# RIVM-bioinformatics/TrueConsense

Hardware: NVIDIA B200
Metric: aligned_bases_per_sec_pileup_consensus (higher is better)
Workload: dtype int32

## Files before the change

trueconsense_b200/csrc/cuda/pileup_warp.cu:

```cuda
#include <limits.h>

#include "pileup_smem.cuh"

namespace {

using namespace tcsm;
constexpr int HI_PLANES = 7;
constexpr int RUN_CAP = 2047;
#ifndef TC_CHUNK_WORDS
#define TC_CHUNK_WORDS 6
#endif
constexpr int CHUNK_WORDS = TC_CHUNK_WORDS;
#ifndef TC_MAX_WARPS
#define TC_MAX_WARPS 24
#endif
#ifndef TC_CIG_PER_WC
#define TC_CIG_PER_WC 15
#endif
#ifndef TC_SEQ_PER_WC
#define TC_SEQ_PER_WC 26
#endif
#ifndef TC_TMA_STAGING
#define TC_TMA_STAGING 1
#endif
#ifndef TC_STAGE_UNROLL
#define TC_STAGE_UNROLL 4
#endif
#ifndef TC_PHASE_WORDS
#define TC_PHASE_WORDS 32
#endif
template <int WC> struct geom {
    static constexpr int ROWW = WC * 8;
    static constexpr int PW = (TC_PHASE_WORDS > 0 && TC_PHASE_WORDS < WC) ? TC_PHASE_WORDS : WC;
    static constexpr int NPH = WC / PW;
    static constexpr int NW = WC / 32;
    static constexpr int RS = PW + 1;
    static constexpr int SEQ_PAD = 4;
    static constexpr int SEQ_CAP = WC * TC_SEQ_PER_WC;
    static constexpr int CIG_CAP = WC * TC_CIG_PER_WC;
    static constexpr int SEQ_WORDS = SEQ_PAD + SEQ_CAP + 8;
    static constexpr int CIG_WORDS = CIG_CAP / 2 + 4;
    static constexpr int WARP_WORDS = 32 * RS + SEQ_WORDS + CIG_WORDS;
    static constexpr int WARPS = (227 * 1024 / 4) / (WARP_WORDS + 2) > TC_MAX_WARPS ? TC_MAX_WARPS : (227 * 1024 / 4) / (WARP_WORDS + 2);
    static constexpr bool TMA = TC_TMA_STAGING && (CIG_CAP + 4 <= 32 * RS);
};

extern __shared__ __align__(16) uint32_t smem[];

struct lane_walk {
    uint32_t cp, cend;
    uint32_t c0, c1;
    uint32_t prev;
    int x, y, rem;
};

template <int ROWW, int CW, bool LIMIT>
__device__ __forceinline__ bool emit_phase(lane_walk& s, const int lq, const uint32_t rowp, const int xlim,
                                           unsigned long long* xi, const int xi_n, const uint32_t sq, int* err) {
    bool any_iter = false;
    while (__any_sync(FULL, (s.cp < s.cend || s.rem > 0) && (!LIMIT || s.x < xlim))) {
        any_iter = true;
        if (s.rem == 0 && s.cp < s.cend && (!LIMIT || s.x < xlim)) {
            uint32_t c = s.c0;
            uint32_t fl = op_flags(c & 15u);
            if (!(fl & 1u)) {
                const uint32_t op = c & 15u;
                const int l = (int)(c >> 4);
                const bool is_d = (op == OP_D);
                const bool ev = is_d || (op == OP_I && (s.prev & 2u));
                const uint32_t col = (uint32_t)min(is_d ? s.x : s.x - 1, xi_n - 1);
                const uint32_t pd = s.prev & 1u;
                red_xi_if(ev, xi, col, is_d ? 1u : 0u - pd, (is_d ? 1u : pd) ^ 1u);
                if (is_d && l > 1) for (int k = s.x + 1; k < min(s.x + l, xi_n); ++k) red_xi_if(true, xi, (uint32_t)k, 1u, 0u);
                s.prev = (fl & 2u) | (is_d ? 1u : 0u);
                if (fl & 2u) s.x += l;
                if (fl & 4u) s.y += l;
                s.cp += 2;
                c = s.c1;
                fl = op_flags(c & 15u);
            }
            if ((fl & 1u) && s.cp < s.cend) {
                const int l = (int)(c >> 4);
                if (s.x + l > ROWW || s.y + l > lq) { atomicCAS(err, 0, TC_ERR_CAPACITY); s.cp = s.cend; }
                else { s.rem = l; s.cp += 2; }
            }
            s.c0 = lds16(s.cp); s.c1 = lds16(s.cp + 2);
        }
        __syncwarp();
        if (s.rem > 0 && (!LIMIT || s.x < xlim)) {
            const int x = s.x;
            const int kb = x & 7;
            const int cl = LIMIT ? min(min(s.rem, 8 * CW - kb), xlim - x) : min(s.rem, 8 * CW - kb);
            {
                const int q0 = (x - kb) + (s.y - x);
                const uint32_t src = sq + (uint32_t)((q0 >> 3) << 2);
                const int sh4 = (q0 & 7) << 2;
                uint32_t w[CW + 1];
#pragma unroll
                for (int j = 0; j <= CW; ++j) w[j] = lds(src + 4 * j);
                const int rem4 = 4 * (kb + cl);
                const uint32_t ro = rowp + (uint32_t)((x >> 3) << 2);
                reds_or(ro, __funnelshift_l(w[1], w[0], sh4) & (0xffffffffu >> (4 * kb)) & ~__funnelshift_rc(0xffffffffu, 0u, rem4));
#pragma unroll
                for (int j = 1; j < CW; ++j)
                    reds_or(ro + 4 * j, __funnelshift_l(w[j + 1], w[j], sh4) & ~__funnelshift_rc(0xffffffffu, 0u, max(rem4 - 32 * j, 0)));
            }
            s.x += cl; s.y += cl; s.rem -= cl;
            s.prev = 2u;
        }
    }
    return any_iter;
}

template <int WC, bool PIECES>
__global__ void __launch_bounds__(geom<WC>::WARPS * 32, 1) warp_pileup_kernel(pileup_args a) {
    using G = geom<WC>;
    constexpr int ROWW = G::ROWW, RS = G::RS, NW = G::NW, NPH = G::NPH, PW = G::PW, KW = G::PW / 32;
    const int lane = threadIdx.x & 31;
    const int L = a.L;
    if (PIECES && a.status->err) return;

    const bool fold = !PIECES && a.span_hint > 0;
    const int ms = PIECES ? PIECE_COLS : ((max(fold ? a.span_hint : a.status->max_span, 1) + 7) & ~7);
    const int slack32 = (256 - ms - 8) & ~7, slack64 = (512 - ms - 8) & ~7, slack128 = (1024 - ms - 8) & ~7;
    const bool mine = (WC == 32) ? (slack32 >= MIN_SLACK)
                    : (WC == 64) ? (slack32 < MIN_SLACK && slack64 >= MIN_SLACK) : (slack64 < MIN_SLACK);
    if (!mine) return;
    const int slack = (WC == 32) ? slack32 : (WC == 64) ? slack64 : slack128;
    if (slack < MIN_SLACK) {
        if (threadIdx.x == 0 && blockIdx.x == 0) atomicCAS(&a.status->err, 0, TC_ERR_CAPACITY);
        return;
    }

    const uint32_t rows = (uint32_t)__cvta_generic_to_shared(smem) + 4u * (threadIdx.x >> 5) * G::WARP_WORDS;
    const uint32_t seq_s = rows + 4u * 32 * RS;
    const uint32_t cig_s = seq_s + 4u * G::SEQ_WORDS;
    for (int i = lane; i < 32 * RS; i += 32) sts(rows + 4 * i, 0u);
    if (lane < G::SEQ_PAD) sts(seq_s + 4 * lane, 0u);
    const uint32_t mbar = (uint32_t)__cvta_generic_to_shared(smem) + 4u * G::WARPS * G::WARP_WORDS + 8u * (threadIdx.x >> 5);
    uint32_t tma_parity = 0;
    if (G::TMA && lane == 0) { mbar_init(mbar, 1); asm volatile("fence.mbarrier_init.release.cluster;" ::: "memory"); }
    __syncwarp();

    const int64_t n_reads = PIECES ? a.n_pieces : a.r.n;
    const int64_t n_seq_words = (int64_t)a.r.seq_off[a.r.n];
    const int64_t n_ops_total = PIECES ? 0 : (int64_t)a.r.cigar_off[a.r.n];
    const int64_t gw = (int64_t)blockIdx.x * G::WARPS + (threadIdx.x >> 5);
    const int64_t n_warps = (int64_t)gridDim.x * G::WARPS;
    int64_t r = gw * n_reads / n_warps;
    const int64_t r_end = (gw + 1) * n_reads / n_warps;

    uint32_t ones[NW], twos[NW], fours[NW], eights[NW], hi[NW][HI_PLANES];
#pragma unroll
    for (int j = 0; j < NW; ++j) {
        ones[j] = twos[j] = fours[j] = eights[j] = 0;
#pragma unroll
        for (int p = 0; p < HI_PLANES; ++p) hi[j][p] = 0;
    }
    int w0 = INT_MIN, run_reads = 0;
    const uint32_t row = rows + 4u * lane * RS;
    int prev_pos = (fold && r > 0 && r < r_end) ? a.r.pos[r - 1] : INT_MIN;
    int my_max_span = 0, my_zero_span = 0;

    auto flush = [&]() {
        __syncwarp();
#pragma unroll
        for (int j = 0; j < NW; ++j) {
            uint32_t planes[4 + HI_PLANES];
            planes[0] = ones[j]; planes[1] = twos[j]; planes[2] = fours[j]; planes[3] = eights[j];
#pragma unroll
            for (int p = 0; p < HI_PLANES; ++p) planes[4 + p] = hi[j][p];
            uint32_t any = 0;
#pragma unroll
            for (int p = 0; p < 4 + HI_PLANES; ++p) any |= planes[p];
            if (any) {
#pragma unroll 4
                for (int bit = 0; bit < 32; ++bit) {
                    if (!((any >> bit) & 1u)) continue;
                    int v = 0;
#pragma unroll
                    for (int p = 0; p < 4 + HI_PLANES; ++p) v |= (int)((planes[p] >> bit) & 1u) << p;
                    const int colr = w0 + 8 * (lane + 32 * j) + (7 - (bit >> 2));
                    const int cls = bit & 3;
                    const int crow = cls == 0 ? TC_ROW_A : cls == 1 ? TC_ROW_C : cls == 2 ? TC_ROW_G : TC_ROW_T;
                    if (colr < L) atomicAdd(&a.counts[(size_t)crow * L + colr], v);
                }
            }
            ones[j] = twos[j] = fours[j] = eights[j] = 0;
#pragma unroll
            for (int p = 0; p < HI_PLANES; ++p) hi[j][p] = 0;
        }
        __syncwarp();
    };

    while (r < r_end) {
        const int nmax = (int)min((int64_t)32, r_end - r);
        const bool valid = lane < nmax;
        const int64_t ri = r + (valid ? lane : 0);
        int p, lq, n, nops_lane, y0 = 0;
        bool passes = true, declined = false;
        uint32_t big = 0;
        uint32_t cs, sq_lane;
        if constexpr (PIECES) {
            const tc_piece* pc = a.pieces + a.piece_order[ri];
            const uint4 m0 = __ldg(reinterpret_cast<const uint4*>(pc)), m1 = __ldg(reinterpret_cast<const uint4*>(pc) + 1);
            p = (int)m0.x; lq = (int)m1.y; y0 = (int)m1.z;
            passes = p < L;
            const uint32_t so = m0.y, co = m0.z;
            nops_lane = (int)m0.w;
            const int p0 = __shfl_sync(FULL, p, 0);
            const bool fresh = (w0 == INT_MIN);
            if (fresh) w0 = max(p0, 0) & ~7;
            const int sv = (int)(((so & 3u) + m1.x + 3u) >> 2), cv = (int)(((co & 3u) + m0.w + 3u) >> 2);
            int s_inc = valid ? sv : 0, c_inc = valid ? cv : 0;
#pragma unroll
            for (int o = 1; o < 32; o <<= 1) {
                const int ts = __shfl_up_sync(FULL, s_inc, o), tc = __shfl_up_sync(FULL, c_inc, o);
                if (lane >= o) { s_inc += ts; c_inc += tc; }
            }
            const bool inwin = p >= w0 && p - w0 < slack;
            const bool fits = valid && inwin && 4 * s_inc <= G::SEQ_CAP && 4 * c_inc <= G::CIG_CAP;
            const unsigned fm = __ballot_sync(FULL, fits);
            n = (fm == FULL) ? 32 : __ffs(~fm) - 1;
            n = min(n, RUN_CAP - run_reads);
            if (n == 0) {
                const bool inwin0 = __shfl_sync(FULL, (int)inwin, 0) != 0;
                if ((!inwin0 && !fresh) || run_reads >= RUN_CAP) {
                    flush();
                    w0 = INT_MIN; run_reads = 0;
                    continue;
                }
                if (lane == 0) atomicCAS(&a.status->err, 0, TC_ERR_CAPACITY);
                r += 1;
                continue;
            }
            const uint32_t sdst = seq_s + 4u * G::SEQ_PAD + 16u * (uint32_t)(s_inc - sv);
            const uint32_t cdst = cig_s + 8u * (uint32_t)(c_inc - cv);
            const int64_t sb_p = (int64_t)(so & ~3u);
            const bool tma_p = G::TMA && __all_sync(FULL, lane >= n || sb_p + 4ll * sv <= n_seq_words);
            if (tma_p) {
                const int s_tot = __shfl_sync(FULL, s_inc, n - 1), c_tot = __shfl_sync(FULL, c_inc, n - 1);
                fence_proxy_async();
                __syncwarp();
                if (lane == 0) mbar_expect_tx(mbar, 16u * (uint32_t)(s_tot + c_tot));
                __syncwarp();
                if (lane < n) {
                    tma_bulk_g2s(sdst, a.r.seq4 + sb_p, 16u * (uint32_t)sv, mbar);
                    if (cv > 0) tma_bulk_g2s(rows + 16u * (uint32_t)(c_inc - cv), a.r.cigar + (co & ~3u), 16u * (uint32_t)cv, mbar);
                }
                mbar_wait(mbar, tma_parity);
                tma_parity ^= 1u;
                const uint32_t sbase = seq_s + 4u * G::SEQ_PAD;
                for (int i = lane; i < s_tot; i += 32) {
                    uint4 v = lds4(sbase + 16 * i);
                    if (multibit(v.x) | multibit(v.y) | multibit(v.z) | multibit(v.w)) {
                        v.x = clear_multibit(v.x); v.y = clear_multibit(v.y); v.z = clear_multibit(v.z); v.w = clear_multibit(v.w);
                    }
                    v.x = __byte_perm(v.x, 0, 0x0123); v.y = __byte_perm(v.y, 0, 0x0123);
                    v.z = __byte_perm(v.z, 0, 0x0123); v.w = __byte_perm(v.w, 0, 0x0123);
                    sts4(sbase + 16 * i, v);
                }
                for (int i = lane; i < c_tot; i += 32) {
                    const uint4 v0 = lds4(rows + 16 * i);
                    big |= v0.x | v0.y | v0.z | v0.w;
                    sts2(cig_s + 8 * i, pack_ops(v0.x, v0.y), pack_ops(v0.z, v0.w));
                    sts4(rows + 16 * i, make_uint4(0u, 0u, 0u, 0u));
                }
            } else {
                if (lane < n) {
                    const int64_t sb = (int64_t)(so & ~3u);
                    constexpr int SB = 4;
                    const bool whole = sb + 4ll * sv <= n_seq_words;
                    for (int v0 = 0; v0 < sv; v0 += SB) {
                        uint4 q[SB];
    #pragma unroll
                        for (int u = 0; u < SB; ++u) {
                            const int v = v0 + u;
                            if (v < sv) {
                                if (whole) q[u] = __ldg(reinterpret_cast<const uint4*>(a.r.seq4 + sb) + v);
                                else {
                                    q[u].x = sb + 4 * v + 0 < n_seq_words ? __ldg(a.r.seq4 + sb + 4 * v + 0) : 0u;
                                    q[u].y = sb + 4 * v + 1 < n_seq_words ? __ldg(a.r.seq4 + sb + 4 * v + 1) : 0u;
                                    q[u].z = sb + 4 * v + 2 < n_seq_words ? __ldg(a.r.seq4 + sb + 4 * v + 2) : 0u;
                                    q[u].w = sb + 4 * v + 3 < n_seq_words ? __ldg(a.r.seq4 + sb + 4 * v + 3) : 0u;
                                }
                            }
                        }
    #pragma unroll
                        for (int u = 0; u < SB; ++u) {
                            const int v = v0 + u;
                            if (v < sv) {
                                if (multibit(q[u].x) | multibit(q[u].y) | multibit(q[u].z) | multibit(q[u].w)) {
                                    q[u].x = clear_multibit(q[u].x); q[u].y = clear_multibit(q[u].y); q[u].z = clear_multibit(q[u].z); q[u].w = clear_multibit(q[u].w);
                                }
                                q[u].x = __byte_perm(q[u].x, 0, 0x0123); q[u].y = __byte_perm(q[u].y, 0, 0x0123);
                                q[u].z = __byte_perm(q[u].z, 0, 0x0123); q[u].w = __byte_perm(q[u].w, 0, 0x0123);
                                sts4(sdst + 16 * v, q[u]);
                            }
                        }
                    }
                    const uint4* csrc = reinterpret_cast<const uint4*>(a.r.cigar + (co & ~3u));
                    for (int v0 = 0; v0 < cv; v0 += 4) {
                        uint4 q[4];
    #pragma unroll
                        for (int u = 0; u < 4; ++u) if (v0 + u < cv) q[u] = __ldg(csrc + v0 + u);
    #pragma unroll
                        for (int u = 0; u < 4; ++u)
                            if (v0 + u < cv) {
                                big |= q[u].x | q[u].y | q[u].z | q[u].w;
                                sts2(cdst + 8 * (v0 + u), pack_ops(q[u].x, q[u].y), pack_ops(q[u].z, q[u].w));
                            }
                    }
                }
            }
            __syncwarp();
            cs = cdst + 2u * (co & 3u);
            if (__any_sync(FULL, big >= OP_BIG)) {
                if (lane < n) {
                    bool after_sat = false;
                    for (uint32_t k = 0; k < m0.w; ++k) {
                        const uint32_t c = __ldg(a.r.cigar + co + k), op = c & 15u;
                        if (c >= OP_BIG) {
                            if (op == OP_H) sts16(cs + 2 * k, (1u << 4) | OP_H);
                            else if (op == OP_S) { sts16(cs + 2 * k, S_SATURATED); after_sat = true; }
                            else declined = true;
                        } else if (after_sat && op_flags(op) != 0u) declined = true;
                    }
                }
                __syncwarp();
            }
            sq_lane = sdst + 4u * (so & 3u);
        } else {
            p = a.r.pos[ri];
            const uint32_t so = a.r.seq_off[ri], so_next = a.r.seq_off[ri + 1];
            const uint32_t co = a.r.cigar_off[ri], co_next = a.r.cigar_off[ri + 1];
            const uint32_t flg = a.r.flag[ri];
            lq = a.r.l_seq[ri];
            passes = !(flg & (a.flag_filter | 4u)) && !(a.ignore_orphans && (flg & 1u) && !(flg & 2u));
            if (a.min_mapq > 0 && a.r.mapq && (int)a.r.mapq[ri] < a.min_mapq) passes = false;
            if (p >= L) {
                if (fold && valid && passes) atomicCAS(&a.status->err, 0, TC_ERR_RANGE);
                passes = false;
            }
            const int p0 = __shfl_sync(FULL, p, 0);
            const bool fresh = (w0 == INT_MIN);
            if (fresh) w0 = max(p0, 0) & ~7;
            const uint32_t sbase_al = __shfl_sync(FULL, so, 0) & ~3u;
            const uint32_t cbase_al = __shfl_sync(FULL, co, 0) & ~3u;
            const bool inwin = p >= w0 && p - w0 < slack;
            const bool fits = valid && inwin && (so_next - sbase_al + 1 <= (uint32_t)G::SEQ_CAP) && (co_next - cbase_al <= (uint32_t)G::CIG_CAP);
            const unsigned fm = __ballot_sync(FULL, fits);
            n = (fm == FULL) ? 32 : __ffs(~fm) - 1;
            n = min(n, RUN_CAP - run_reads);
            if (n == 0) {
                const bool inwin0 = __shfl_sync(FULL, (int)inwin, 0) != 0;
                if ((!inwin0 && !fresh) || run_reads >= RUN_CAP) {
                    flush();
                    w0 = INT_MIN; run_reads = 0;
                    continue;
                }
                if (inwin0 && lane == 0) atomicCAS(&a.status->err, 0, TC_ERR_CAPACITY);
                if (fold && lane == 0) {
                    if (p0 < prev_pos) atomicCAS(&a.status->err, 0, TC_ERR_UNSORTED);
                    if (p0 < 0 && passes) atomicCAS(&a.status->err, 0, TC_ERR_RANGE);
                }
                prev_pos = p0;
                r += 1;
                continue;
            }

            {
                const uint32_t send = __shfl_sync(FULL, so_next, n - 1) + 1;
                const int nv = (int)((send - sbase_al + 3) >> 2);
                const uint32_t cend = __shfl_sync(FULL, co_next, n - 1);
                const int ncv = (int)((cend - cbase_al + 3) >> 2);
                uint32_t dirty = 0;
                const uint32_t sdst = seq_s + 4u * G::SEQ_PAD;
                uint32_t exmin = 1u;
                const bool use_tma = G::TMA && (int64_t)sbase_al + 4ll * nv <= n_seq_words && (int64_t)cbase_al + 4ll * ncv <= n_ops_total;
                if (use_tma) {
                    fence_proxy_async();
                    __syncwarp();
                    if (lane == 0) {
                        mbar_expect_tx(mbar, 16u * (uint32_t)(nv + ncv));
                        tma_bulk_g2s(sdst, a.r.seq4 + sbase_al, 16u * (uint32_t)nv, mbar);
                        if (ncv > 0) tma_bulk_g2s(rows, a.r.cigar + cbase_al, 16u * (uint32_t)ncv, mbar);
                    }
                }
                {
                    const int64_t s_lo = ((int64_t)send - 1) & ~3ll, s_len = (int64_t)send - sbase_al;
                    const int64_t c_lo = (int64_t)cend & ~3ll, c_len = (int64_t)cend - cbase_al;
                    if (lane == 0) {
                        const int64_t sw = min(s_len + 4, n_seq_words - s_lo) & ~3ll, cw = min(c_len + 4, n_ops_total - c_lo) & ~3ll;
                        if (sw > 0) prefetch_l2_bulk(a.r.seq4 + s_lo, (uint32_t)(4 * sw));
                        if (cw > 0) prefetch_l2_bulk(a.r.cigar + c_lo, (uint32_t)(4 * cw));
                    }
                    const int64_t rm = r + n + 64;
                    if (rm < n_reads) {
                        if (lane == 0) prefetch_l2(a.r.pos + rm);
                        if (lane == 1) prefetch_l2(a.r.seq_off + rm);
                        if (lane == 2) prefetch_l2(a.r.cigar_off + rm);
                        if (lane == 3) prefetch_l2(a.r.l_seq + rm);
                        if (lane == 4) prefetch_l2(a.r.flag + rm);
                    }
                }
                if (use_tma) {
                    mbar_wait(mbar, tma_parity);
                    tma_parity ^= 1u;
                    for (int i = lane; i < nv; i += 32) {
                        uint4 v = lds4(sdst + 16 * i);
                        if (multibit(v.x) | multibit(v.y) | multibit(v.z) | multibit(v.w)) {
                            v.x = clear_multibit(v.x); v.y = clear_multibit(v.y); v.z = clear_multibit(v.z); v.w = clear_multibit(v.w);
                        }
                        v.x = __byte_perm(v.x, 0, 0x0123); v.y = __byte_perm(v.y, 0, 0x0123);
                        v.z = __byte_perm(v.z, 0, 0x0123); v.w = __byte_perm(v.w, 0, 0x0123);
                        sts4(sdst + 16 * i, v);
                    }
                    for (int i = lane; i < ncv; i += 32) {
                        const uint4 v0 = lds4(rows + 16 * i);
                        exmin = min(exmin, min(min(op_exotic_min(v0.x), op_exotic_min(v0.y)), min(op_exotic_min(v0.z), op_exotic_min(v0.w))));
                        big |= v0.x | v0.y | v0.z | v0.w;
                        sts2(cig_s + 8 * i, pack_ops(v0.x, v0.y), pack_ops(v0.z, v0.w));
                        sts4(rows + 16 * i, make_uint4(0u, 0u, 0u, 0u));
                    }
                } else {
                    if ((int64_t)sbase_al + 4ll * nv <= n_seq_words) {
                        const uint4* src = reinterpret_cast<const uint4*>(a.r.seq4 + sbase_al);
                        int t = 0;
                        constexpr int SU = TC_STAGE_UNROLL;
                        for (int i = lane; i < nv; i += 32 * SU, t += SU) {
                            uint4 v[SU];
        #pragma unroll
                            for (int u = 0; u < SU; ++u) if (i + 32 * u < nv) v[u] = __ldg(src + i + 32 * u);
        #pragma unroll
                            for (int u = 0; u < SU; ++u) if (i + 32 * u < nv) {
                                const uint32_t z = multibit(v[u].x) | multibit(v[u].y) | multibit(v[u].z) | multibit(v[u].w);
                                dirty |= (z != 0 ? 1u : 0u) << (t + u);
                                v[u].x = __byte_perm(v[u].x, 0, 0x0123); v[u].y = __byte_perm(v[u].y, 0, 0x0123);
                                v[u].z = __byte_perm(v[u].z, 0, 0x0123); v[u].w = __byte_perm(v[u].w, 0, 0x0123);
                                sts4(sdst + 16 * (i + 32 * u), v[u]);
                            }
                        }
                    } else {
                        int t = 0;
                        for (int i = lane; i < nv; i += 32, ++t) {
                            uint32_t w[4];
        #pragma unroll
                            for (int u = 0; u < 4; ++u) {
                                const int64_t wi = (int64_t)sbase_al + 4 * i + u;
                                w[u] = wi < n_seq_words ? __ldg(a.r.seq4 + wi) : 0u;
                            }
                            const uint32_t z = multibit(w[0]) | multibit(w[1]) | multibit(w[2]) | multibit(w[3]);
                            dirty |= (z != 0 ? 1u : 0u) << t;
        #pragma unroll
                            for (int u = 0; u < 4; ++u) sts(sdst + 16 * i + 4 * u, __byte_perm(w[u], 0, 0x0123));
                        }
                    }
                    if ((int64_t)cbase_al + 4ll * ncv <= n_ops_total) {
                        const uint4* csrc = reinterpret_cast<const uint4*>(a.r.cigar + cbase_al);
                        for (int i = lane; i < ncv; i += 64) {
                            uint4 v0 = __ldg(csrc + i), v1 = make_uint4(16u, 16u, 16u, 16u);
                            const bool b1 = i + 32 < ncv;
                            if (b1) v1 = __ldg(csrc + i + 32);
                            exmin = min(exmin, min(min(op_exotic_min(v0.x), op_exotic_min(v0.y)), min(op_exotic_min(v0.z), op_exotic_min(v0.w))));
                            exmin = min(exmin, min(min(op_exotic_min(v1.x), op_exotic_min(v1.y)), min(op_exotic_min(v1.z), op_exotic_min(v1.w))));
                            big |= v0.x | v0.y | v0.z | v0.w | v1.x | v1.y | v1.z | v1.w;
                            sts2(cig_s + 8 * i, pack_ops(v0.x, v0.y), pack_ops(v0.z, v0.w));
                            if (b1) sts2(cig_s + 8 * (i + 32), pack_ops(v1.x, v1.y), pack_ops(v1.z, v1.w));
                        }
                    } else {
                        for (int i = lane; i < 4 * ncv; i += 32) {
                            const int64_t oi = (int64_t)cbase_al + i;
                            const uint32_t c = oi < n_ops_total ? __ldg(a.r.cigar + oi) : 16u;
                            exmin = min(exmin, op_exotic_min(c));
                            big |= c;
                            sts16(cig_s + 2 * i, c);
                        }
                    }
                }
                declined = exmin == 0u;
                __syncwarp();
                if (__any_sync(FULL, big >= OP_BIG)) {
                    if (lane < n) {
                        bool after_sat = false;
                        for (uint32_t k = co; k < co_next; ++k) {
                            const uint32_t c = __ldg(a.r.cigar + k), op = c & 15u;
                            if (c >= OP_BIG) {
                                if (op == OP_H) sts16(cig_s + 2 * (k - cbase_al), (1u << 4) | OP_H);
                                else if (op == OP_S) { sts16(cig_s + 2 * (k - cbase_al), S_SATURATED); after_sat = true; }
                                else declined = true;
                            } else if (after_sat && op_flags(op) != 0u) declined = true;
                        }
                    }
                    __syncwarp();
                }
                while (__any_sync(FULL, dirty != 0)) {
                    if (dirty) {
                        const int t = __ffs(dirty) - 1;
                        dirty &= dirty - 1;
                        const uint32_t q = sdst + 16 * (lane + 32 * t);
                        uint4 v = lds4(q);
                        v.x = clear_multibit(v.x); v.y = clear_multibit(v.y); v.z = clear_multibit(v.z); v.w = clear_multibit(v.w);
                        sts4(q, v);
                    }
                }
                __syncwarp();
            }
            cs = cig_s + 2u * (co - cbase_al);
            nops_lane = (int)(co_next - co);
            sq_lane = seq_s + 4u * G::SEQ_PAD + 4u * (so - sbase_al);
        }
        const bool act = lane < n && passes;
        const int nops = act ? nops_lane : 0;
        const int x0 = p - w0;
        const uint32_t sq = act ? sq_lane : seq_s + 4u * G::SEQ_PAD;
        if (!act) cs = cig_s;
        if (__any_sync(FULL, act && lq == 0)) {
            if (act && lq == 0)
                for (int k = 0; k < nops; ++k) {
                    const uint32_t c = lds16(cs + 2 * k);
                    if (op_flags(c & 15u) & 1u) sts16(cs + 2 * k, (c & ~15u) | OP_N);
                }
            __syncwarp();
        }
        const bool skip = __any_sync(FULL, declined);
        if (skip && lane == 0) atomicCAS(&a.status->err, 0, TC_ERR_CAPACITY);
        lane_walk st;
        st.cp = cs; st.cend = cs + 2u * (uint32_t)(skip ? 0 : nops);
        st.c0 = lds16(cs); st.c1 = lds16(cs + 2);
        st.prev = 0; st.x = x0; st.y = y0; st.rem = 0;
#pragma unroll
        for (int ph = 0; ph < NPH; ++ph) {
            const int xlim = (ph == NPH - 1) ? INT_MAX : 8 * PW * (ph + 1);
            const bool did = emit_phase<ROWW, CHUNK_WORDS, (NPH > 1)>(st, lq, row - 4u * PW * ph, xlim, a.xi + w0, L - w0, sq, &a.status->err);
            __syncwarp();
            if (!did) continue;
#pragma unroll
            for (int k = 0; k < KW; ++k) {
                const int j = ph * KW + k;
                const uint32_t col = rows + 4u * (lane + 32 * k);
#pragma unroll
                for (int blk = 0; blk < 2; ++blk) {
                    if (blk * 16 < n) {
                        uint32_t xw[16];
#pragma unroll
                        for (int q = 0; q < 16; ++q) { xw[q] = lds(col + 4u * (blk * 16 + q) * RS); sts(col + 4u * (blk * 16 + q) * RS, 0u); }
                        uint32_t twosA, twosB, foursA, foursB, eightsA, eightsB, sixteens;
                        csa(twosA, ones[j], ones[j], xw[0], xw[1]);
                        csa(twosB, ones[j], ones[j], xw[2], xw[3]);
                        csa(foursA, twos[j], twos[j], twosA, twosB);
                        csa(twosA, ones[j], ones[j], xw[4], xw[5]);
                        csa(twosB, ones[j], ones[j], xw[6], xw[7]);
                        csa(foursB, twos[j], twos[j], twosA, twosB);
                        csa(eightsA, fours[j], fours[j], foursA, foursB);
                        csa(twosA, ones[j], ones[j], xw[8], xw[9]);
                        csa(twosB, ones[j], ones[j], xw[10], xw[11]);
                        csa(foursA, twos[j], twos[j], twosA, twosB);
                        csa(twosA, ones[j], ones[j], xw[12], xw[13]);
                        csa(twosB, ones[j], ones[j], xw[14], xw[15]);
                        csa(foursB, twos[j], twos[j], twosA, twosB);
                        csa(eightsB, fours[j], fours[j], foursA, foursB);
                        csa(sixteens, eights[j], eights[j], eightsA, eightsB);
                        uint32_t carry = sixteens;
#pragma unroll
                        for (int pl = 0; pl < HI_PLANES; ++pl) { const uint32_t t = hi[j][pl] & carry; hi[j][pl] ^= carry; carry = t; }
                    }
                }
            }
            __syncwarp();
        }
        const int x_end = st.x;

        if (fold) {
            int pprev = __shfl_up_sync(FULL, p, 1);
            if (lane == 0) pprev = prev_pos;
            if (lane < n && p < pprev) atomicCAS(&a.status->err, 0, TC_ERR_UNSORTED);
            prev_pos = __shfl_sync(FULL, p, n - 1);
            const int span = act ? x_end - x0 : 0;
            const bool bad = act && (p >= L || p + span > L);
            if (bad) atomicCAS(&a.status->err, 0, TC_ERR_RANGE);
            const bool has = act && span > 0 && !bad;
            my_max_span = max(my_max_span, span);
            my_zero_span += (act && span == 0) ? 1 : 0;
            const unsigned g0 = __match_any_sync(FULL, has ? p : -1 - lane);
            if (has && (__ffs(g0) - 1) == lane) atomicAdd(&a.diff[p], __popc(g0));
            const unsigned g1 = __match_any_sync(FULL, has ? p + span : -1 - lane);
            if (has && (__ffs(g1) - 1) == lane) atomicAdd(&a.diff[p + span], -__popc(g1));
        }

        r += n;
        run_reads += n;
    }
    if (run_reads > 0) flush();
    if (fold) {
        my_max_span = __reduce_max_sync(FULL, my_max_span);
        my_zero_span = __reduce_add_sync(FULL, my_zero_span);
        if (lane == 0) {
            if (my_max_span > 0) atomicMax(&a.status->max_span, my_max_span);
            if (my_zero_span > 0) atomicAdd(&a.status->n_zero_span, my_zero_span);
        }
    }
}

}

bool tc_pileup_warp_supported(const pileup_args& a) {
    return (((uintptr_t)a.r.seq4 | (uintptr_t)a.r.cigar) & 15u) == 0;
}

template <int WC, bool PIECES>
static int launch_geom(tc_ctx* ctx, const pileup_args& a, cudaStream_t s) {
    using G = geom<WC>;
    const size_t smem = sizeof(uint32_t) * (size_t)(G::WARP_WORDS + 2) * G::WARPS;
    const uint32_t bit = 1u << ((WC == 32 ? 0 : WC == 64 ? 1 : 2) + (PIECES ? 3 : 0));
    if (!(ctx->warp_attr_set & bit)) {
        TC_CUDA(cudaFuncSetAttribute(warp_pileup_kernel<WC, PIECES>, cudaFuncAttributeMaxDynamicSharedMemorySize, (int)smem));
        ctx->warp_attr_set |= bit;
    }
    warp_pileup_kernel<WC, PIECES><<<ctx->sm_count, G::WARPS * 32, smem, s>>>(a);
    TC_LAUNCH_CHECK();
    return TC_OK;
}

int tc_pileup_warp_launch(tc_ctx* ctx, const pileup_args& a, cudaStream_t s) {
    if (a.span_hint > 0) {
        const int wc = warp_geometry(a.span_hint);
        if (wc == 32) return launch_geom<32, false>(ctx, a, s);
        if (wc == 64) return launch_geom<64, false>(ctx, a, s);
        return launch_geom<128, false>(ctx, a, s);
    }
    int rc = launch_geom<32, false>(ctx, a, s);
    if (rc) return rc;
    rc = launch_geom<64, false>(ctx, a, s);
    if (rc) return rc;
    return launch_geom<128, false>(ctx, a, s);
}

int tc_pileup_warp_launch_pieces(tc_ctx* ctx, const pileup_args& a, cudaStream_t s) { return launch_geom<64, true>(ctx, a, s); }
```

Baseline: 1229 billion.

## Group reads by CIGAR length via warp bitonic sort to balance lane walks

In the non-piece path with WC==64, reads are now handled in groups of up to 128 within a window. Each group is bitonic-sorted in registers by CIGAR op count, so the 32 reads processed together have similar walk lengths and lanes diverge less. Because the reads of a batch are no longer contiguous, each one's sequence and CIGAR data are packed into shared memory at prefix-sum offsets, copied by each lane with direct __ldg loads by default (per-lane TMA behind a flag). The cost is extra sort and shuffle work, gather loads in place of one bulk TMA copy, and the sortedness check moved to group setup.

```diff
diff --git a/trueconsense_b200/csrc/cuda/pileup_warp.cu b/trueconsense_b200/csrc/cuda/pileup_warp.cu
--- a/trueconsense_b200/csrc/cuda/pileup_warp.cu
+++ b/trueconsense_b200/csrc/cuda/pileup_warp.cu
@@ -29,6 +29,13 @@
 #ifndef TC_PHASE_WORDS
 #define TC_PHASE_WORDS 32
 #endif
+#ifndef TC_GROUP_READS
+#define TC_GROUP_READS 128
+#endif
+#ifndef TC_GROUP_LDG
+#define TC_GROUP_LDG 2
+#endif
+static_assert(TC_GROUP_READS % 32 == 0 && TC_GROUP_READS <= 256, "a group is whole register slots of 32 reads, ranks fit 8 bits");
 template <int WC> struct geom {
     static constexpr int ROWW = WC * 8;
     static constexpr int PW = (TC_PHASE_WORDS > 0 && TC_PHASE_WORDS < WC) ? TC_PHASE_WORDS : WC;
@@ -193,10 +200,158 @@
         __syncwarp();
     };
 
+    constexpr int GS = TC_GROUP_READS / 32;
+    constexpr bool GROUPED = !PIECES && WC == 64 && G::TMA && GS > 1;
+    uint32_t g_rank[GS > 0 ? GS : 1];
+    int64_t g_r0 = 0, plain_end = r;
+    int g_len = 0, g_next = 0;
+
+    auto normalise_tma = [&](int nv, int ncv, uint32_t& exmin, uint32_t& big) {
+        mbar_wait(mbar, tma_parity);
+        tma_parity ^= 1u;
+        const uint32_t sdst = seq_s + 4u * G::SEQ_PAD;
+        for (int i = lane; i < nv; i += 32) {
+            uint4 v = lds4(sdst + 16 * i);
+            if (multibit(v.x) | multibit(v.y) | multibit(v.z) | multibit(v.w)) {
+                v.x = clear_multibit(v.x); v.y = clear_multibit(v.y); v.z = clear_multibit(v.z); v.w = clear_multibit(v.w);
+            }
+            v.x = __byte_perm(v.x, 0, 0x0123); v.y = __byte_perm(v.y, 0, 0x0123);
+            v.z = __byte_perm(v.z, 0, 0x0123); v.w = __byte_perm(v.w, 0, 0x0123);
+            sts4(sdst + 16 * i, v);
+        }
+        for (int i = lane; i < ncv; i += 32) {
+            const uint4 v0 = lds4(rows + 16 * i);
+            exmin = min(exmin, min(min(op_exotic_min(v0.x), op_exotic_min(v0.y)), min(op_exotic_min(v0.z), op_exotic_min(v0.w))));
+            big |= v0.x | v0.y | v0.z | v0.w;
+            sts2(cig_s + 8 * i, pack_ops(v0.x, v0.y), pack_ops(v0.z, v0.w));
+            sts4(rows + 16 * i, make_uint4(0u, 0u, 0u, 0u));
+        }
+    };
+
     while (r < r_end) {
-        const int nmax = (int)min((int64_t)32, r_end - r);
+        if constexpr (GROUPED) {
+            if (g_len == 0 && r >= plain_end) {
+                const bool fresh = (w0 == INT_MIN);
+                const int wg = fresh ? (max(a.r.pos[r], 0) & ~7) : w0;
+                const int gmax = (int)min((int64_t)TC_GROUP_READS, r_end - r);
+                int glen = min(gmax, RUN_CAP - run_reads);
+                int pk[GS];
+                uint32_t key[GS];
+#pragma unroll
+                for (int s = 0; s < GS; ++s) {
+                    const int64_t i = r + 32 * s + lane;
+                    bool ok = false;
+                    pk[s] = INT_MAX; key[s] = 0;
+                    if (32 * s + lane < gmax) {
+                        const int pi = a.r.pos[i];
+                        const uint32_t so = a.r.seq_off[i], so_next = a.r.seq_off[i + 1];
+                        const uint32_t co = a.r.cigar_off[i], co_next = a.r.cigar_off[i + 1];
+                        const uint32_t sv = (so_next + 4u - (so & ~3u)) >> 2, cv = (co_next + 3u - (co & ~3u)) >> 2;
+                        ok = pi >= wg && pi - wg < slack && 4 * sv <= (uint32_t)G::SEQ_CAP && 4 * cv <= (uint32_t)G::CIG_CAP &&
+                             (int64_t)(so & ~3u) + 4ll * sv <= n_seq_words && (int64_t)(co & ~3u) + 4ll * cv <= n_ops_total;
+                        pk[s] = pi;
+                        key[s] = min(co_next - co, 0xfffffeu);
+                    }
+                    const unsigned bad = __ballot_sync(FULL, !ok);
+                    if (bad) glen = min(glen, 32 * s + __ffs(bad) - 1);
+                }
+                if (glen == 0) {
+                    const int pf = __shfl_sync(FULL, pk[0], 0);
+                    if (run_reads >= RUN_CAP || (!fresh && !(pf >= wg && pf - wg < slack))) {
+                        flush();
+                        w0 = INT_MIN; run_reads = 0;
+                        continue;
+                    }
+                }
+                uint32_t kmin = UINT_MAX, kmax = 0;
+#pragma unroll
+                for (int s = 0; s < GS; ++s) {
+                    const bool in = 32 * s + lane < glen;
+                    kmin = min(kmin, in ? key[s] : UINT_MAX);
+                    kmax = max(kmax, in ? key[s] : 0u);
+                    g_rank[s] = ((in ? key[s] : 0xffffffu) << 8) | (uint32_t)(32 * s + lane);
+                }
+                kmin = __reduce_min_sync(FULL, kmin);
+                kmax = __reduce_max_sync(FULL, kmax);
+                if (glen <= 32 || kmin == kmax) {
+                    plain_end = r + max(glen, 1);
+                } else {
+                    w0 = wg;
+#pragma unroll
+                    for (int k = 2; k <= 32 * GS; k <<= 1) {
+#pragma unroll
+                        for (int j = k >> 1; j > 0; j >>= 1) {
+                            if (j >= 32) {
+#pragma unroll
+                                for (int s = 0; s < GS; ++s) {
+                                    const int t = s | (j >> 5);
+                                    if (t == s) continue;
+                                    const bool up = ((32 * s) & k) == 0;
+                                    const uint32_t lo = min(g_rank[s], g_rank[t]), hi = max(g_rank[s], g_rank[t]);
+                                    g_rank[s] = up ? lo : hi;
+                                    g_rank[t] = up ? hi : lo;
+                                }
+                            } else {
+#pragma unroll
+                                for (int s = 0; s < GS; ++s) {
+                                    const uint32_t o = __shfl_xor_sync(FULL, g_rank[s], j);
+                                    const bool up = ((32 * s + lane) & k) == 0;
+                                    g_rank[s] = (up == ((lane & j) == 0)) ? min(g_rank[s], o) : max(g_rank[s], o);
+                                }
+                            }
+                        }
+                    }
+                    int plast = 0;
+#pragma unroll
+                    for (int s = 0; s < GS; ++s) {
+                        int pp = __shfl_up_sync(FULL, pk[s], 1);
+                        const int carry = s > 0 ? __shfl_sync(FULL, pk[s > 0 ? s - 1 : 0], 31) : prev_pos;
+                        if (lane == 0) pp = carry;
+                        if (fold && 32 * s + lane < glen && pk[s] < pp) atomicCAS(&a.status->err, 0, TC_ERR_UNSORTED);
+                        const int t = __shfl_sync(FULL, pk[s], (glen - 1) & 31);
+                        if (s == (glen - 1) >> 5) plast = t;
+                    }
+                    prev_pos = plast;
+                    g_r0 = r; g_len = glen; g_next = 0;
+                    if (lane == 0) {
+                        const int64_t s_lo = a.r.seq_off[r] & ~3u, c_lo = a.r.cigar_off[r] & ~3u;
+                        const int64_t s_len = (int64_t)a.r.seq_off[r + glen] + 1 - s_lo, c_len = (int64_t)a.r.cigar_off[r + glen] - c_lo;
+                        const int64_t sw = min(2 * s_len + 4, n_seq_words - s_lo) & ~3ll, cw = min(2 * c_len + 4, n_ops_total - c_lo) & ~3ll;
+                        if (sw > 0) prefetch_l2_bulk(a.r.seq4 + s_lo, (uint32_t)(4 * sw));
+                        if (cw > 0) prefetch_l2_bulk(a.r.cigar + c_lo, (uint32_t)(4 * cw));
+                    }
+#pragma unroll
+                    for (int s = 0; s < GS; ++s) {
+                        const int64_t rm = r + glen + 64 + 32 * s;
+                        if (rm < n_reads) {
+                            if (lane == 0) prefetch_l2(a.r.pos + rm);
+                            if (lane == 1) prefetch_l2(a.r.seq_off + rm);
+                            if (lane == 2) prefetch_l2(a.r.cigar_off + rm);
+                            if (lane == 3) prefetch_l2(a.r.l_seq + rm);
+                            if (lane == 4) prefetch_l2(a.r.flag + rm);
+                        }
+                    }
+                }
+            }
+        }
+        const bool grouped = GROUPED && g_len > 0;
+        int nmax;
+        int64_t ri;
+        if (grouped) {
+            const int q = g_next + lane;
+            uint32_t v = 0;
+#pragma unroll
+            for (int s = 0; s < GS; ++s) {
+                const uint32_t t = __shfl_sync(FULL, g_rank[s], q & 31);
+                if (s == (q >> 5)) v = t;
+            }
+            nmax = min(32, g_len - g_next);
+            ri = g_r0 + (lane < nmax ? (int)(v & 255u) : 0);
+        } else {
+            nmax = (int)min((int64_t)32, r_end - r);
+            ri = r + (lane < nmax ? lane : 0);
+        }
         const bool valid = lane < nmax;
-        const int64_t ri = r + (valid ? lane : 0);
         int p, lq, n, nops_lane, y0 = 0;
         bool passes = true, declined = false;
         uint32_t big = 0;
@@ -342,13 +497,25 @@
                 if (fold && valid && passes) atomicCAS(&a.status->err, 0, TC_ERR_RANGE);
                 passes = false;
             }
+            int sv = 0, cv = 0, s_inc = 0, c_inc = 0;
+            if (grouped) {
+                sv = (int)((so_next + 4u - (so & ~3u)) >> 2);
+                cv = (int)((co_next + 3u - (co & ~3u)) >> 2);
+                s_inc = valid ? sv : 0; c_inc = valid ? cv : 0;
+#pragma unroll
+                for (int o = 1; o < 32; o <<= 1) {
+                    const int ts = __shfl_up_sync(FULL, s_inc, o), tc = __shfl_up_sync(FULL, c_inc, o);
+                    if (lane >= o) { s_inc += ts; c_inc += tc; }
+                }
+            }
             const int p0 = __shfl_sync(FULL, p, 0);
             const bool fresh = (w0 == INT_MIN);
             if (fresh) w0 = max(p0, 0) & ~7;
             const uint32_t sbase_al = __shfl_sync(FULL, so, 0) & ~3u;
             const uint32_t cbase_al = __shfl_sync(FULL, co, 0) & ~3u;
             const bool inwin = p >= w0 && p - w0 < slack;
-            const bool fits = valid && inwin && (so_next - sbase_al + 1 <= (uint32_t)G::SEQ_CAP) && (co_next - cbase_al <= (uint32_t)G::CIG_CAP);
+            const bool fits = grouped ? valid && 4 * s_inc <= G::SEQ_CAP && 4 * c_inc <= G::CIG_CAP
+                                      : valid && inwin && (so_next - sbase_al + 1 <= (uint32_t)G::SEQ_CAP) && (co_next - cbase_al <= (uint32_t)G::CIG_CAP);
             const unsigned fm = __ballot_sync(FULL, fits);
             n = (fm == FULL) ? 32 : __ffs(~fm) - 1;
             n = min(n, RUN_CAP - run_reads);
@@ -369,14 +536,64 @@
                 continue;
             }
 
-            {
+            uint32_t exmin = 1u;
+            if (grouped) {
+                const uint32_t sdst = seq_s + 4u * G::SEQ_PAD + 16u * (uint32_t)(s_inc - sv);
+#if TC_GROUP_LDG
+                if (lane < n) {
+                    const uint4* ssrc = reinterpret_cast<const uint4*>(a.r.seq4 + (so & ~3u));
+                    for (int v0 = 0; v0 < sv; v0 += TC_GROUP_LDG) {
+                        uint4 q[TC_GROUP_LDG];
+#pragma unroll
+                        for (int u = 0; u < TC_GROUP_LDG; ++u) if (v0 + u < sv) q[u] = __ldg(ssrc + v0 + u);
+#pragma unroll
+                        for (int u = 0; u < TC_GROUP_LDG; ++u)
+                            if (v0 + u < sv) {
+                                if (multibit(q[u].x) | multibit(q[u].y) | multibit(q[u].z) | multibit(q[u].w)) {
+                                    q[u].x = clear_multibit(q[u].x); q[u].y = clear_multibit(q[u].y); q[u].z = clear_multibit(q[u].z); q[u].w = clear_multibit(q[u].w);
+                                }
+                                q[u].x = __byte_perm(q[u].x, 0, 0x0123); q[u].y = __byte_perm(q[u].y, 0, 0x0123);
+                                q[u].z = __byte_perm(q[u].z, 0, 0x0123); q[u].w = __byte_perm(q[u].w, 0, 0x0123);
+                                sts4(sdst + 16 * (v0 + u), q[u]);
+                            }
+                    }
+                    const uint4* csrc = reinterpret_cast<const uint4*>(a.r.cigar + (co & ~3u));
+                    const uint32_t cdst = cig_s + 8u * (uint32_t)(c_inc - cv);
+                    for (int v0 = 0; v0 < cv; v0 += TC_GROUP_LDG) {
+                        uint4 q[TC_GROUP_LDG];
+#pragma unroll
+                        for (int u = 0; u < TC_GROUP_LDG; ++u) if (v0 + u < cv) q[u] = __ldg(csrc + v0 + u);
+#pragma unroll
+                        for (int u = 0; u < TC_GROUP_LDG; ++u)
+                            if (v0 + u < cv) {
+                                exmin = min(exmin, min(min(op_exotic_min(q[u].x), op_exotic_min(q[u].y)), min(op_exotic_min(q[u].z), op_exotic_min(q[u].w))));
+                                big |= q[u].x | q[u].y | q[u].z | q[u].w;
+                                sts2(cdst + 8 * (v0 + u), pack_ops(q[u].x, q[u].y), pack_ops(q[u].z, q[u].w));
+                            }
+                    }
+                }
+#else
+                const int s_tot = __shfl_sync(FULL, s_inc, n - 1), c_tot = __shfl_sync(FULL, c_inc, n - 1);
+                fence_proxy_async();
+                __syncwarp();
+                if (lane == 0) mbar_expect_tx(mbar, 16u * (uint32_t)(s_tot + c_tot));
+                __syncwarp();
+                if (lane < n) {
+                    tma_bulk_g2s(sdst, a.r.seq4 + (so & ~3u), 16u * (uint32_t)sv, mbar);
+                    if (cv > 0) tma_bulk_g2s(rows + 16u * (uint32_t)(c_inc - cv), a.r.cigar + (co & ~3u), 16u * (uint32_t)cv, mbar);
+                }
+                normalise_tma(s_tot, c_tot, exmin, big);
+#endif
+                __syncwarp();
+                cs = cig_s + 8u * (uint32_t)(c_inc - cv) + 2u * (co & 3u);
+                sq_lane = sdst + 4u * (so & 3u);
+            } else {
                 const uint32_t send = __shfl_sync(FULL, so_next, n - 1) + 1;
                 const int nv = (int)((send - sbase_al + 3) >> 2);
                 const uint32_t cend = __shfl_sync(FULL, co_next, n - 1);
                 const int ncv = (int)((cend - cbase_al + 3) >> 2);
                 uint32_t dirty = 0;
                 const uint32_t sdst = seq_s + 4u * G::SEQ_PAD;
-                uint32_t exmin = 1u;
                 const bool use_tma = G::TMA && (int64_t)sbase_al + 4ll * nv <= n_seq_words && (int64_t)cbase_al + 4ll * ncv <= n_ops_total;
                 if (use_tma) {
                     fence_proxy_async();
@@ -405,24 +622,7 @@
                     }
                 }
                 if (use_tma) {
-                    mbar_wait(mbar, tma_parity);
-                    tma_parity ^= 1u;
-                    for (int i = lane; i < nv; i += 32) {
-                        uint4 v = lds4(sdst + 16 * i);
-                        if (multibit(v.x) | multibit(v.y) | multibit(v.z) | multibit(v.w)) {
-                            v.x = clear_multibit(v.x); v.y = clear_multibit(v.y); v.z = clear_multibit(v.z); v.w = clear_multibit(v.w);
-                        }
-                        v.x = __byte_perm(v.x, 0, 0x0123); v.y = __byte_perm(v.y, 0, 0x0123);
-                        v.z = __byte_perm(v.z, 0, 0x0123); v.w = __byte_perm(v.w, 0, 0x0123);
-                        sts4(sdst + 16 * i, v);
-                    }
-                    for (int i = lane; i < ncv; i += 32) {
-                        const uint4 v0 = lds4(rows + 16 * i);
-                        exmin = min(exmin, min(min(op_exotic_min(v0.x), op_exotic_min(v0.y)), min(op_exotic_min(v0.z), op_exotic_min(v0.w))));
-                        big |= v0.x | v0.y | v0.z | v0.w;
-                        sts2(cig_s + 8 * i, pack_ops(v0.x, v0.y), pack_ops(v0.z, v0.w));
-                        sts4(rows + 16 * i, make_uint4(0u, 0u, 0u, 0u));
-                    }
+                    normalise_tma(nv, ncv, exmin, big);
                 } else {
                     if ((int64_t)sbase_al + 4ll * nv <= n_seq_words) {
                         const uint4* src = reinterpret_cast<const uint4*>(a.r.seq4 + sbase_al);
@@ -478,22 +678,7 @@
                         }
                     }
                 }
-                declined = exmin == 0u;
                 __syncwarp();
-                if (__any_sync(FULL, big >= OP_BIG)) {
-                    if (lane < n) {
-                        bool after_sat = false;
-                        for (uint32_t k = co; k < co_next; ++k) {
-                            const uint32_t c = __ldg(a.r.cigar + k), op = c & 15u;
-                            if (c >= OP_BIG) {
-                                if (op == OP_H) sts16(cig_s + 2 * (k - cbase_al), (1u << 4) | OP_H);
-                                else if (op == OP_S) { sts16(cig_s + 2 * (k - cbase_al), S_SATURATED); after_sat = true; }
-                                else declined = true;
-                            } else if (after_sat && op_flags(op) != 0u) declined = true;
-                        }
-                    }
-                    __syncwarp();
-                }
                 while (__any_sync(FULL, dirty != 0)) {
                     if (dirty) {
                         const int t = __ffs(dirty) - 1;
@@ -505,10 +690,25 @@
                     }
                 }
                 __syncwarp();
-            }
-            cs = cig_s + 2u * (co - cbase_al);
+                cs = cig_s + 2u * (co - cbase_al);
+                sq_lane = seq_s + 4u * G::SEQ_PAD + 4u * (so - sbase_al);
+            }
+            declined = exmin == 0u;
+            if (__any_sync(FULL, big >= OP_BIG)) {
+                if (lane < n) {
+                    bool after_sat = false;
+                    for (uint32_t k = co; k < co_next; ++k) {
+                        const uint32_t c = __ldg(a.r.cigar + k), op = c & 15u;
+                        if (c >= OP_BIG) {
+                            if (op == OP_H) sts16(cs + 2 * (k - co), (1u << 4) | OP_H);
+                            else if (op == OP_S) { sts16(cs + 2 * (k - co), S_SATURATED); after_sat = true; }
+                            else declined = true;
+                        } else if (after_sat && op_flags(op) != 0u) declined = true;
+                    }
+                }
+                __syncwarp();
+            }
             nops_lane = (int)(co_next - co);
-            sq_lane = seq_s + 4u * G::SEQ_PAD + 4u * (so - sbase_al);
         }
         const bool act = lane < n && passes;
         const int nops = act ? nops_lane : 0;
@@ -572,10 +772,12 @@
         const int x_end = st.x;
 
         if (fold) {
-            int pprev = __shfl_up_sync(FULL, p, 1);
-            if (lane == 0) pprev = prev_pos;
-            if (lane < n && p < pprev) atomicCAS(&a.status->err, 0, TC_ERR_UNSORTED);
-            prev_pos = __shfl_sync(FULL, p, n - 1);
+            if (!grouped) {
+                int pprev = __shfl_up_sync(FULL, p, 1);
+                if (lane == 0) pprev = prev_pos;
+                if (lane < n && p < pprev) atomicCAS(&a.status->err, 0, TC_ERR_UNSORTED);
+                prev_pos = __shfl_sync(FULL, p, n - 1);
+            }
             const int span = act ? x_end - x0 : 0;
             const bool bad = act && (p >= L || p + span > L);
             if (bad) atomicCAS(&a.status->err, 0, TC_ERR_RANGE);
@@ -588,7 +790,12 @@
             if (has && (__ffs(g1) - 1) == lane) atomicAdd(&a.diff[p + span], -__popc(g1));
         }
 
-        r += n;
+        if (grouped) {
+            g_next += n;
+            if (g_next == g_len) { r += g_len; g_len = 0; }
+        } else {
+            r += n;
+        }
         run_reads += n;
     }
     if (run_reads > 0) flush();
```

Result: slower. 775.1 billion (median of 6 runs) (-36.9%).
